# neel-dey/anatomix

Measured on AMD Instinct MI355X. Metric: 128^3 volumes/sec feature-extraction (6M UNet), higher is better.
Workload: dtype f16; 1 GPU; anatomix 6M UNet (ngf=16,num_downs=4) forward on sw_batch=4 windows of 1x128^3 (the predictor call of sliding_window_inference, BASELINE configs[1] / the metric); fp32 NCDHW in/out, 16-bit (f16) channels-last activations, fp32 accumulate; holds the 1e-3 tolerance against the fp32 reference in rel-L2 ONLY (max-norm 0.86e-3 .. 1.4e-3 by weight seed; the mode that holds both norms is value_strict); batch_per_gpu=4, window=128, parallelism=replicas x1 (no data-path collective)

## Files before the change

anatomix_amd/_lib.py:

```python
from __future__ import annotations

import ctypes as C
import os

_HERE = os.path.dirname(os.path.abspath(__file__))
LIB_PATH = os.environ.get("AMX_LIB_PATH") or os.path.join(_HERE, "csrc", "libanatomix_amd.so")

NORM = {"none": 0, "batch": 1, "instance": 2, "instance_affine": 3}
ACT = {"none": 0, "relu": 1, "lrelu": 2}
POOL = {"Max": 0, "Avg": 1}
INTERP = {"nearest": 0, "trilinear": 1}
WARP = {"bilinear": 0, "nearest": 1}
SEG_LABEL = {"float32": 0, "int64": 1, "uint8": 2}
SW_MAP = {"constant": 0, "gaussian": 1}
SW_OUT = {"features": 0, "logits": 1, "labels": 2}
PRECISION = {"f16": 0, "fp16": 0, "float16": 0, "bf16": 1, "bfloat16": 1, "f16x2": 2, "bf16x2": 3, "strict": 3, "fp32": 3,
             "f16x2mx": 4, "strict_mx": 4}


class UnetCfg(C.Structure):
    _fields_ = [
        ("input_nc", C.c_int32), ("output_nc", C.c_int32), ("num_downs", C.c_int32), ("ngf", C.c_int32),
        ("norm", C.c_int32), ("norm_eps", C.c_float), ("activation", C.c_int32), ("act_slope", C.c_float),
        ("final_act", C.c_int32), ("pooling", C.c_int32), ("interp", C.c_int32), ("doubleconv", C.c_int32),
# ... 62 lines not shown
    "amx_sliding_window_workspace_bytes": (C.c_size_t, [_P, _I, _I, _I, _I]),
    "amx_sliding_window": (_I, [_P, _P, _I, _I, _I, _I, _I, _I, C.c_double, _I, C.c_double, _I, _I, _P, _P, _I, _P, _P, _P, _P,
                                C.c_size_t, _P]),
    "amx_conv3d_packed_bytes": (C.c_size_t, [_I, _I]),
    "amx_conv3d_k3_reflect": (_I, [_P, _I, _P, _I, _P, _P, _P, _I, _I, _I, _I, _I, _I, C.c_float, _I, _P, _P, _P, _P]),
    "amx_conv3d_k3_reflect_probe": (_I, [_P, _I, _P, _I, _P, _P, _P, _I, _I, _I, _I, _I, _I, C.c_float, _I, _P, _P, _P, _P, _P, _P, _P, _P]),
    "amx_conv3d_dgrad_interior_supported": (_I, [_I, _I, _I, _I, _I, _I]),
    "amx_conv3d_dgrad_interior": (_I, [_P, _I, _P, _I, _I, _I, _I, _I, _I, _I, _I, _I, _P, _P, _P]),
    "amx_conv3d_dgrad_shell_scratch_bytes": (C.c_size_t, []),
    "amx_conv3d_dgrad_fold_shell": (_I, [_P, _I, _P, _I, _I, _P, _I, _I, _I, _I, _I, _I, _P, _P]),
    "amx_conv3d_pack_batch": (_I, [C.POINTER(PackReq), _I, _I, _P]),
    "amx_conv3d_scratch_bytes": (C.c_size_t, [_I, _I, _I, _I, _I, _I, _I, _I]),
    "amx_conv3d_k3_reflect_ws": (_I, [_P, _I, _P, _I, _P, _P, _P, _I, _I, _I, _I, _I, _I, C.c_float, _I, _P, _P, _P, _P, C.c_size_t, _P]),
    "amx_conv3d_upcat_merged_packed_bytes": (C.c_size_t, [_I, _I, _I]),
    "amx_conv3d_upcat_merged": (_I, [_P, _I, _P, _I, _P, _P, _P, _I, _I, _I, _I, _I, _I, C.c_float, _I, _P, _P, _P, _P]),
    "amx_conv3d_k3_reflect_ex": (_I, [_P, _I, _P, _I, _P, _I, _I, _I, _P, _P, _I, _I, _I, _I, _I, _I, C.c_float, _I, _P, _P, _P, _P]),
    "amx_pool2": (_I, [_P, _P, _I, _I, _I, _I, _I, _I, _I, _P]),
    "amx_instance_norm_scratch_bytes": (C.c_size_t, [_I, _I]),
    "amx_instance_norm": (_I, [_P, _P, _P, C.c_float, _I, C.c_longlong, _I, _I, C.c_float, _P, _I, _P]),
    "amx_upsample2_trilinear": (_I, [_P, _P, _I, _I, _I, _I, _I, _I, _P]),
    "amx_upsample2_trilinear_backward": (_I, [_P, _P, _I, _I, _I, _I, _I, _I, _P]),
    "amx_upcat_split_backward": (_I, [_P, _P, _P, _I, _I, _I, _I, _I, _I, _I, _I, _P]),
    "amx_upcat_split_backward_framed": (_I, [_P, _P, _P, _I, _I, _I, _I, _I, _I, _I, _I, _P]),
    "amx_export_ncdhw": (_I, [_P, _I, _I, _I, _I, _I, _P, _I, _P]),
    "amx_import_ncdhw": (_I, [_P, _P, _I, _I, _I, _I, _I, C.c_longlong, C.c_longlong, C.c_longlong, C.c_longlong, _I, _I, _P]),
    "amx_train_scratch_bytes": (C.c_size_t, [_I]),
    "amx_bn_train_forward": (_I, [_P, _P, _P, _P, C.c_float, _I, C.c_longlong, _I, _I, C.c_float, _P, _P, _P, _P, _P,
                                  C.c_float, _I, _P]),
    "amx_bn_act_backward": (_I, [_P, _P, _P, _P, _P, _P, _P, _P, _P, _I, _I, _I, _I, _I, _I, C.c_float, _P, _I, _P]),
    "amx_bn_act_backward_recompute": (_I, [_P, _P, _P, _P, _P, _P, _P, _P, _P, _I, _I, _I, _I, _I, _I, C.c_float, _P, _I, _P]),
# ... 183 lines not shown
```

anatomix_amd/csrc/amx_api.hip:

```cpp
#include <stdarg.h>
#include <stdio.h>
#include <string.h>

#include <string>
#include <vector>

#include "amx_gemm.h"
#include "amx_launch.h"

static thread_local std::string g_err;

int amx::fail(int code, const char* fmt, ...) {
  char buf[512];
  va_list ap;
  va_start(ap, fmt);
  vsnprintf(buf, sizeof buf, fmt, ap);
  va_end(ap);
  g_err = buf;
  return code;
}

using namespace amx;

extern "C" {
// ... 258 lines not shown
                       precision, d_wpk, d_out16, d_out32, stream);
}

int amx_conv3d_k3_reflect_ex(const void* d_x0, int c0, const void* d_x1, int c1, const float* d_weight, int weight_mode,
                             int cin_real, int cout_real, const float* d_scale, const float* d_shift, int cout, int n,
                             int d, int hh, int w, int act, float slope, int precision, void* d_wpk, void* d_out16,
                             float* d_out32, void* stream) {
  return conv3d_single(d_x0, c0, d_x1, c1, d_weight, weight_mode, cin_real, cout_real, d_scale, d_shift, cout, n, d, hh, w,
                       act, slope, precision, d_wpk, d_out16, d_out32, stream);
}

size_t amx_conv3d_upcat_merged_packed_bytes(int c0, int c1, int cout) {
  return 2 * (align_up((size_t)cout * c0 * 28 * 2, 256) + amx::conv_upmerge_packed_bytes(c1, cout, 0));
}

int amx_conv3d_upcat_merged(const void* d_x0, int c0, const void* d_x1, int c1, const float* d_weight, const float* d_scale,
                            const float* d_shift, int cout, int n, int d, int hh, int w, int act, float slope, int precision,
                            void* d_wpk, void* d_partial, void* d_out16, void* stream) {
  if (!d_x0 || !d_x1 || !d_weight || !d_wpk || !d_partial || !d_out16) return fail(AMX_ERR_INVALID, "null argument");
  if (precision < AMX_PREC_F16 || precision > AMX_PREC_BF16X2) return fail(AMX_ERR_INVALID, "unsupported precision %d", precision);
  const bool split = is_split(precision);
  if (c0 != cout || !amx::conv_upmerge_eligible(c0, c1, cout, d, hh, w, 1, split))
    return fail(AMX_ERR_INVALID, "merged concat conv needs c0 == cout >= 32 (16 in the strict precisions), c1 %% 32 == 0, w >= 16, even dims "
                "(c0=%d c1=%d cout=%d dims %d,%d,%d)", c0, c1, cout, d, hh, w);
  hipStream_t st = (hipStream_t)stream;
  const int q = amx::conv_pick_q(cout, w, precision);
  char* wmerge = (char*)d_wpk + align_up((size_t)cout * c0 * 28 * 2 * (split ? 2 : 1), 256);
  AMX_HIP(amx::launch_pack_weights(d_weight, d_scale, d_wpk, c0, c0, cout, q, precision, st, 0, 0, c0 + c1));
  AMX_HIP(amx::launch_pack_upmerge(d_weight, d_scale, wmerge, c0, c0 + c1, c1, cout, precision, st));
  amx::ConvParams p;
  memset(&p, 0, sizeof p);
  p.N = n; p.D = d; p.H = hh; p.W = w; p.Cout = cout;
  amx::set_src0(p, d_x0, c0, d, hh, w, precision);
  p.wpk = (const char*)d_wpk; p.act = AMX_ACT_NONE;
  amx::set_out(p, d_partial, cout, d, hh, w, precision);
  AMX_HIP(amx::launch_conv(p, precision, q, st));
  amx::UpmergeParams u;
  memset(&u, 0, sizeof u);
  amx::set_src(u, d_x1, c1, d / 2, hh / 2, w / 2, precision);
  u.N = n; u.LD = d / 2; u.LH = hh / 2; u.LW = w / 2; u.Cout = cout;
  u.wpk = wmerge; u.part = (const char*)d_partial; u.out = (char*)d_out16;
  u.bias = d_shift; u.act = act; u.slope = slope;
  AMX_HIP(amx::launch_conv_upmerge(u, precision, st));
  return AMX_OK;
}

int amx_pool2(const void* d_in, void* d_out, int n, int dout, int hout, int wout, int c, int avg, int precision,
              void* stream) {
  if (!d_in || !d_out || c % 8) return fail(AMX_ERR_INVALID, "bad argument");
  AMX_HIP(amx::launch_pool2(d_in, d_out, n, dout, hout, wout, c, avg, precision, (hipStream_t)stream));
  return AMX_OK;
}

size_t amx_train_scratch_bytes(int c) { return amx::train_scratch_bytes(c); }

int amx_bn_train_forward(const void* d_x, void* d_y, const float* d_gamma, const float* d_beta, float eps, int n,
                         long long voxels, int c, int act, float slope, void* d_scratch, float* d_save_mean,
                         float* d_save_rstd, float* d_running_mean, float* d_running_var, float momentum, int precision,
                         void* stream) {
// ... 600 lines not shown
```

anatomix_amd/csrc/amx_common.h:

```cpp
#pragma once
#include <hip/hip_runtime.h>
#include <stdint.h>
#include <stdlib.h>

namespace amx {

typedef _Float16 f16;
typedef __bf16 bf16;
typedef __attribute__((ext_vector_type(8))) _Float16 f16x8;
typedef __attribute__((ext_vector_type(8))) __bf16 bf16x8;
typedef __attribute__((ext_vector_type(4))) float f32x4;

constexpr int kSteps = 14;

__host__ __device__ constexpr int tapA_index(int s) {
  return s < 9 ? s * 3 : (s < 12 ? (s - 9) * 9 + 2 : (s == 12 ? 8 : 26));
}
__host__ __device__ constexpr int tapB_index(int s) {
  return s < 9 ? s * 3 + 1 : (s < 12 ? (s - 9) * 9 + 5 : (s == 12 ? 17 : -1));
}

enum Act { ACT_NONE = 0, ACT_RELU = 1, ACT_LRELU = 2 };

struct DeviceOnce {
// ... 64 lines not shown
}

struct UpmergeParams {
  const char* src;
  long long sn, sz, sy, sx;
  int C1;
  int N, LD, LH, LW, Cout;
  const char* wpk;
  const char* part;
  char* out;
  const float* bias;
  int act;
  float slope;
  int nbz, nby, nbx;
  int* oflow;
  int dbg;
  int cs, ocs;
};

constexpr int MLP_MAXB = 8;

struct WgradParams {
  const char* dy;
  long long yn, yz, yy, yx;
  const char* src0;
  long long s0n, s0z, s0y, s0x;
  const char* src1;
  long long s1n, s1z, s1y, s1x;
  int C0, C1, up_shift;
  int N, D, H, W, Cout;
  float* partial;
// ... 9 lines not shown
```

anatomix_amd/csrc/amx_conv3d_upmerge.hip:

```cpp
#include <stdlib.h>

#include "amx_device.h"
#include "amx_launch.h"

namespace amx {


template <int Q, int TZ, int TY, int NBUF, int KS, bool SPLIT = false, int LXT = 16>
struct UpmCfg {
  static_assert(LXT == 16 || LXT == 8, "a tile is 16 cells of one low-res row, or 8 cells of two rows (rows shorter than 16)");
  static constexpr int RPT = 16 / LXT;
  static constexpr int BY = TY * RPT;
  static constexpr int NP = SPLIT ? 2 : 1;
  static_assert(!SPLIT || KS == 1, "strict precision: 32-channel stages");
  static constexpr int T = TZ * TY;
  static constexpr int HZ = TZ + 2, HY = BY + 2, HX = LXT + 2, HV = HZ * HY * HX;
  static constexpr int PL = ((HV * 16 + 255) / 256) * 256;
  static constexpr int BUF = 4 * KS * NP * PL;
  static constexpr int NJ = (HV + 63) / 64;
  static constexpr int NDMA = 4 * KS * NP * NJ;
  static constexpr int PER_WAVE = (NDMA + 7) / 8;
  static constexpr int LDS_BYTES = NBUF * BUF;
  static_assert(LDS_BYTES <= 160 * 1024, "ring must fit the LDS");
};

template <typename T_, int Q, int TZ, int TY, int NBUF, int KS, bool SPLIT, int LXT>
__global__ __launch_bounds__(512) void conv3d_upmerge_kernel(const UpmergeParams p) {
  typedef UpmCfg<Q, TZ, TY, NBUF, KS, SPLIT, LXT> C;
  constexpr int RPT = C::RPT, BY = C::BY;
  constexpr int NP = C::NP;
  typedef typename Ops<T_>::vec8 vec8;
  constexpr int HY = C::HY, HX = C::HX, PL = C::PL, NT = C::T;
  extern __shared__ __attribute__((aligned(16))) char smem[];

  const int tid = threadIdx.x, lane = tid & 63;
  const int wave = __builtin_amdgcn_readfirstlane(tid >> 6);
  const int li = lane & 15, g = lane >> 4;
  const int lix = li & (LXT - 1), liy = LXT == 8 ? li >> 3 : 0;
  const int pz = wave >> 2, py = (wave >> 1) & 1, px = wave & 1;

  const int nbricks = p.nbz * p.nby * p.nbx * p.N;
  const int ncg = p.Cout / (16 * Q);
  const int items = nbricks * ncg;
  const int G = gridDim.x;
  int jw = blockIdx.x;
  if ((G & 7) == 0) jw = (jw & 7) * (G >> 3) + (jw >> 3);
  const int it0 = (int)((long long)items * jw / G), it1 = (int)((long long)items * (jw + 1) / G);
  const int nstage = p.C1 / (32 * KS);
  const int T_total = (it1 - it0) * nstage;
  if (T_total <= 0) return;

  struct Item { int bx, by, bz, n, cg; };
  auto decode = [&](int it) {
    Item r;
    r.cg = it / nbricks;
    int b = it - r.cg * nbricks;
    r.bx = b % p.nbx; b /= p.nbx;
    r.by = b % p.nby; b /= p.nby;
    r.bz = b % p.nbz;
    r.n = b / p.nbz;
    return r;
  };

  int dma_item = -1;
  int off[C::PER_WAVE];
  auto issue = [&](int it, int stage, int bsel) {
    const Item I = decode(it);
    if (it != dma_item) {
      dma_item = it;
#pragma unroll
      for (int m = 0; m < C::PER_WAVE; ++m) {
        const int id = wave + 8 * m;
        const int j = id % C::NJ;
        const int hv = j * 64 + lane;
        const int hz = hv / (HY * HX), rem = hv - hz * (HY * HX), hy = rem / HX, hx = rem - hy * HX;
        int gz = I.bz * TZ - 1 + hz, gy = I.by * BY - 1 + hy, gx = I.bx * LXT - 1 + hx;
        gz = gz < 0 ? 0 : (gz >= p.LD ? p.LD - 1 : gz);
        gy = gy < 0 ? 0 : (gy >= p.LH ? p.LH - 1 : gy);
        gx = gx < 0 ? 0 : (gx >= p.LW ? p.LW - 1 : gx);
        off[m] = hv < C::HV ? gz * (int)p.sz + gy * (int)p.sy + gx * (int)p.sx : -1;
      }
    }
    const char* base = p.src + (long long)I.n * p.sn;
    const int cs = p.cs ? p.cs : 32;
    char* buf = smem + bsel * C::BUF;
#pragma unroll
    for (int m = 0; m < C::PER_WAVE; ++m) {
      const int id = wave + 8 * m;
      if (id < C::NDMA) {
        const int plane = id / C::NJ, j = id - plane * C::NJ;
        const int cbyte = stage * (64 * KS) + (SPLIT && plane >= 4 ? p.C1 * 2 + (plane - 4) * 16 : plane * 16);
        if (off[m] >= 0)
          dma16_asm(base + off[m] + (long long)(cbyte >> 5) * cs + (cbyte & 31),
                    (unsigned)__builtin_amdgcn_readfirstlane((int)lds_addr(buf + plane * PL + j * 1024)));
      }
    }
  };

  auto wptr = [&](int it, int stage) -> const char* {
    const int cg = it / nbricks;
    return p.wpk + ((((long long)cg * nstage * KS + stage * KS) * 8 + wave) * 8 * NP * Q) * 1024 + lane * 16;
  };
  auto woff = [](const int e2) { return ((e2 >> 3) * 64 + (e2 & 7)) * NP * Q * 1024; };
  constexpr int NTAP = 8 * KS;
  constexpr int WIN = 4;
  vec8 wq[WIN][NP][Q];
  const int lbase = g * PL + ((pz * HY + py + liy) * HX + px + lix) * 16;

  f32x4 acc[NT][Q];
  int nx_it = it0, nx_stage = 0;
  auto step_next = [&]() {
    if (++nx_stage == nstage) { nx_stage = 0; ++nx_it; }
  };
  issue(nx_it, nx_stage, 0);
  step_next();
  if (NBUF > 2 && T_total > 1) { issue(nx_it, nx_stage, 1); step_next(); }
  {
    const char* w0 = wptr(it0, 0);
#pragma unroll
    for (int e = 0; e < WIN; ++e)
#pragma unroll
      for (int h = 0; h < NP; ++h)
#pragma unroll
        for (int q = 0; q < Q; ++q) wq[e][h][q] = *(const vec8*)(w0 + woff(e) + (h * Q + q) * 1024);
  }

  int cu_it = it0, cu_stage = 0;
  bool bad = false;
  unsigned pend[NT][2 * Q * NP];
  int pend_it = -1;
  unsigned padd[NT][2 * Q * NP];
  auto load_part = [&](const int it) {
    const Item I = decode(it);
    const int lx = I.bx * LXT + lix;
    const int ocs = p.ocs ? p.ocs : 32, cb2 = (I.cg * 16 * Q + g * 4 * Q) * 2;
    const long long sy = (long long)p.Cout * 2 * NP * (2 * p.LW), sz = sy * (2 * p.LH), sx = ocs == 32 ? (long long)p.Cout * 2 * NP : 32;
    const char* pb = p.part + (long long)I.n * sz * (2 * p.LD) + pz * sz + py * sy + (2 * lx + px) * sx + (long long)(cb2 >> 5) * ocs + (cb2 & 31);
#pragma unroll
    for (int i = 0; i < NT; ++i) {
      const int lz = I.bz * TZ + i / TY, ly = I.by * BY + (i % TY) * RPT + liy;
      const bool in = (lz < p.LD) & (ly < p.LH) & (lx < p.LW);
#pragma unroll
      for (int hl = 0; hl < NP; ++hl) {
        const char* src = pb + 2 * lz * sz + 2 * ly * sy + hl * p.Cout * 2;
        unsigned* dst = &padd[i][hl * 2 * Q];
        if (Q == 1) {
          const uint2 v = in ? *(const uint2*)src : make_uint2(0u, 0u);
          dst[0] = v.x; dst[1] = v.y;
        } else {
#pragma unroll
          for (int h = 0; h < Q / 2; ++h) {
            const uint4 v = in ? *(const uint4*)(src + h * 16) : make_uint4(0u, 0u, 0u, 0u);
            dst[4 * h] = v.x; dst[4 * h + 1] = v.y; dst[4 * h + 2] = v.z; dst[4 * h + 3] = v.w;
          }
        }
      }
    }
  };
  auto flush = [&]() {
    const Item I = decode(pend_it);
    pend_it = -1;
    const int lx = I.bx * LXT + lix;
    const int ocs = p.ocs ? p.ocs : 32, cb2 = (I.cg * 16 * Q + g * 4 * Q) * 2;
    const long long sy = (long long)p.Cout * 2 * NP * (2 * p.LW), sz = sy * (2 * p.LH), sx = ocs == 32 ? (long long)p.Cout * 2 * NP : 32;
    char* pb = p.out + (long long)I.n * sz * (2 * p.LD) + pz * sz + py * sy + (2 * lx + px) * sx + (long long)(cb2 >> 5) * ocs + (cb2 & 31);
#pragma unroll
    for (int i = 0; i < NT; ++i) {
      const int lz = I.bz * TZ + i / TY, ly = I.by * BY + (i % TY) * RPT + liy;
      if (lz >= p.LD || ly >= p.LH || lx >= p.LW) continue;
#pragma unroll
      for (int hl = 0; hl < NP; ++hl) {
        char* dst = pb + 2 * lz * sz + 2 * ly * sy + hl * p.Cout * 2;
        const unsigned* v = &pend[i][hl * 2 * Q];
        if (Q == 1) *(uint2*)dst = make_uint2(v[0], v[1]);
        else {
#pragma unroll
          for (int h = 0; h < Q / 2; ++h) *(uint4*)(dst + h * 16) = make_uint4(v[4 * h], v[4 * h + 1], v[4 * h + 2], v[4 * h + 3]);
        }
      }
    }
  };
  for (int t = 0; t < T_total; ++t) {
    if (t == 0) asm volatile("s_waitcnt vmcnt(0)" ::: "memory");
    else asm volatile("" ::"v"(wq[0][0][0]) : "memory");
    __syncthreads();
    if (t + NBUF - 1 < T_total && !(p.dbg & 1)) {
      issue(nx_it, nx_stage, (t + NBUF - 1) % NBUF);
      step_next();
    }
    if (pend_it >= 0 && !(p.dbg & 4)) flush();
    if (cu_stage == nstage - 1 && !(p.dbg & 16)) load_part(cu_it);
    const char* buf = smem + (t % NBUF) * C::BUF + lbase;
    if (cu_stage == 0) {
#pragma unroll
      for (int i = 0; i < NT; ++i)
#pragma unroll
        for (int q = 0; q < Q; ++q) acc[i][q] = f32x4{0.f, 0.f, 0.f, 0.f};
    }
    const bool more = t + 1 < T_total;
    const int w_it = cu_stage + 1 < nstage ? cu_it : cu_it + 1, w_stage = cu_stage + 1 < nstage ? cu_stage + 1 : 0;
    const char* wn = more ? wptr(w_it, w_stage) : p.wpk;
    const char* wc = wptr(cu_it, cu_stage);
    if (!(p.dbg & 2)) {
      constexpr int GT = SPLIT ? 2 : (NT < 4 ? NT : 4), NGT = NT / GT, NG = NTAP * NGT;
      vec8 fb[2][GT][NP];
      auto load_group = [&](const int gi, const int set) {
        const int e2 = gi / NGT, i0 = (gi % NGT) * GT;
        const int ks = e2 >> 3, ez = (e2 >> 2) & 1, ey = (e2 >> 1) & 1, ex = e2 & 1;
#pragma unroll
        for (int k = 0; k < GT; ++k) {
          const int lz = (i0 + k) / TY, ly = (i0 + k) % TY;
#pragma unroll
          for (int h = 0; h < NP; ++h)
            fb[set][k][h] = *(const vec8*)(buf + (ks + h) * 4 * PL + (((lz + ez) * HY + ly * RPT + ey) * HX + ex) * 16);
        }
      };
      load_group(0, 0);
#pragma unroll
// ... 12 lines not shown
            }
          }
        __builtin_amdgcn_sched_barrier(0);
        if ((gi % NGT) == NGT - 1 && (e + WIN < NTAP || more)) {
          const char* src = e + WIN < NTAP ? wc + woff(e + WIN) : wn + woff(e + WIN - NTAP);
#pragma unroll
          for (int h = 0; h < NP; ++h)
#pragma unroll
            for (int q = 0; q < Q; ++q) wq[e % WIN][h][q] = *(const vec8*)(src + (h * Q + q) * 1024);
        }
      }
    }
    if (++cu_stage < nstage) continue;
    cu_stage = 0;

    {
      const int cgb = (cu_it / nbricks) * 16 * Q + g * 4 * Q;
      auto cvt = [](const unsigned w, const int half) { return (float)__builtin_bit_cast(T_, (unsigned short)(half ? w >> 16 : w & 0xffffu)); };
#pragma unroll
      for (int q = 0; q < Q; ++q) {
        const f32x4 bv = p.bias ? *(const f32x4*)(p.bias + cgb + q * 4) : f32x4{0.f, 0.f, 0.f, 0.f};
#pragma unroll
        for (int i = 0; i < NT; ++i)
#pragma unroll
          for (int j = 0; j < 4; ++j) {
            float a = cvt(padd[i][2 * q + (j >> 1)], j & 1);
            if (SPLIT) a += cvt(padd[i][2 * Q + 2 * q + (j >> 1)], j & 1);
            acc[i][q][j] += bv[j] + a;
          }
      }
      act_inplace<NT * Q>(&acc[0][0], p.act, p.slope);
    }
#pragma unroll
    for (int i = 0; i < NT; ++i)
#pragma unroll
      for (int q = 0; q < Q; ++q) {
#pragma unroll
        for (int j = 0; j < 4; ++j)
          if (RangeCheck<T_>::on) bad |= RangeCheck<T_>::bad(acc[i][q][j]);
        pend[i][2 * q] = (unsigned)to_bits<T_>(acc[i][q][0]) | ((unsigned)to_bits<T_>(acc[i][q][1]) << 16);
        pend[i][2 * q + 1] = (unsigned)to_bits<T_>(acc[i][q][2]) | ((unsigned)to_bits<T_>(acc[i][q][3]) << 16);
        if (SPLIT) {
          float r[4];
#pragma unroll
          for (int j = 0; j < 4; ++j) r[j] = acc[i][q][j] - (float)(T_)acc[i][q][j];
          pend[i][2 * Q + 2 * q] = (unsigned)to_bits<T_>(r[0]) | ((unsigned)to_bits<T_>(r[1]) << 16);
          pend[i][2 * Q + 2 * q + 1] = (unsigned)to_bits<T_>(r[2]) | ((unsigned)to_bits<T_>(r[3]) << 16);
        }
      }
    pend_it = cu_it;
    ++cu_it;
  }
  if (pend_it >= 0 && !(p.dbg & 4)) flush();
  if (RangeCheck<T_>::on) raise_flag(p.oflow, bad);
}

template <typename T>
__global__ void pack_upmerge_kernel(const float* __restrict__ w, const float* __restrict__ scale, T* __restrict__ wpk, int c_off,
                                    int CinTotal, int C1, int Cout, int Q, int split) {
  const int nstage = C1 / 32, NP = split ? 2 : 1;
  const long long total = (long long)(Cout / (16 * Q)) * nstage * 64 * NP * Q * 512;
  for (long long idx = blockIdx.x * (long long)blockDim.x + threadIdx.x; idx < total; idx += (long long)gridDim.x * blockDim.x) {
    const int j = idx & 7, lane = (idx >> 3) & 63;
    long long r = idx >> 9;
    const int q = r % Q; r /= Q;
    const int part = r % NP; r /= NP;
    const int e = r % 8; r /= 8;
    const int cls = r % 8; r /= 8;
// ... 16 lines not shown
    const float v = sum * (scale ? scale[cout] : 1.f);
    const T vh = (T)v;
    wpk[idx] = part ? (T)(v - (float)vh) : vh;
  }
}

size_t conv_upmerge_packed_bytes(int C1, int Cout, int split) { return (size_t)Cout * C1 * 64 * 2 * (split ? 2 : 1); }
size_t conv_upmerge_partial_bytes(int N, int D, int H, int W, int Cout) { return (size_t)N * D * H * W * Cout * 2; }
int conv_upmerge_q(int Cout, int split) { return (!split && Cout % 32 == 0) ? 2 : 1; }

bool conv_upmerge_eligible(int C0, int C1, int Cout, int D, int H, int W, int up_shift, int split) {
  return up_shift == 1 && C0 >= 16 && C1 >= 32 && C1 % 32 == 0 && Cout >= (split ? 16 : 32) && Cout % 16 == 0 && W >= 16 && !(D & 1) && !(H & 1) &&
         !(W & 1) && D >= 4 && H >= 4;
}

template <typename T, int Q, int TZ, int TY, int NBUF, int KS, bool SPLIT = false, int LXT = 16>
static hipError_t launch_upm(UpmergeParams p, hipStream_t st, ConvLaunchInfo* info) {
  typedef UpmCfg<Q, TZ, TY, NBUF, KS, SPLIT, LXT> C;
  if (info)
    info->report(0, "conv3d_upmerge<%s,q%d,%dx%dx%d,b%d,k%d>", __is_same(T, f16) ? (SPLIT ? "f16x2" : "f16") : (SPLIT ? "bf16x2" : "bf16"), Q,
                 TZ, C::BY, LXT, NBUF, 32 * KS);
  auto kern = conv3d_upmerge_kernel<T, Q, TZ, TY, NBUF, KS, SPLIT, LXT>;
  static amx::DeviceOnce attr_once;
  if (!attr_once.done()) {
    hipError_t e = hipFuncSetAttribute((const void*)kern, hipFuncAttributeMaxDynamicSharedMemorySize, C::LDS_BYTES);
    if (e != hipSuccess) return e;
    attr_once.set();
  }
  const int cus = device_cus(attr_once.dev);
  if (cus == 0) return hipErrorUnknown;
  p.nbz = (p.LD + TZ - 1) / TZ;
  p.nby = (p.LH + C::BY - 1) / C::BY;
  p.nbx = (p.LW + LXT - 1) / LXT;
  const long long items = (long long)p.nbz * p.nby * p.nbx * p.N * (p.Cout / (16 * Q));
  const long long grid = items < cus ? items : cus;
  hipLaunchKernelGGL(kern, dim3((unsigned)grid), dim3(512), C::LDS_BYTES, st, p);
  return hipGetLastError();
}

template <typename T>
static hipError_t launch_upm_split(const UpmergeParams& p, hipStream_t st, ConvLaunchInfo* info) {
  if (p.LW < 16) return launch_upm<T, 1, 2, 2, 3, 1, true, 8>(p, st, info);
  const long long cells = (long long)p.N * p.LD * p.LH * ((p.LW + 15) / 16);
  if (cells / 8 * (p.Cout / 16) >= 256) return launch_upm<T, 1, 2, 4, 2, 1, true>(p, st, info);
  return launch_upm<T, 1, 2, 2, 3, 1, true>(p, st, info);
}

template <typename T>
static hipError_t launch_upm_t(const UpmergeParams& p, hipStream_t st, ConvLaunchInfo* info) {
  const int Q = conv_upmerge_q(p.Cout, 0);
  if (p.LW < 16) {
    if (Q == 2) return p.C1 % 64 == 0 ? launch_upm<T, 2, 2, 2, 2, 2, false, 8>(p, st, info) : launch_upm<T, 2, 2, 2, 3, 1, false, 8>(p, st, info);
// ... 36 lines not shown
```

include/anatomix_amd.h:

```cpp
#ifndef ANATOMIX_AMD_H
#define ANATOMIX_AMD_H

#include <stddef.h>
#include <stdint.h>

#ifdef __cplusplus
extern "C" {
#endif

#define AMX_VERSION 100

typedef enum amx_status {
  AMX_OK = 0,
  AMX_ERR_INVALID = -1,
  AMX_ERR_SHAPE = -2,
  AMX_ERR_NOT_LOADED = -3,
  AMX_ERR_WORKSPACE = -4,
  AMX_ERR_HIP = -5,
  AMX_ERR_OVERFLOW = -6
} amx_status;

enum { AMX_NORM_NONE = 0, AMX_NORM_BATCH_EVAL = 1, AMX_NORM_INSTANCE = 2, AMX_NORM_INSTANCE_AFFINE = 3 };
enum { AMX_ACT_NONE = 0, AMX_ACT_RELU = 1, AMX_ACT_LRELU = 2 };
enum { AMX_POOL_MAX = 0, AMX_POOL_AVG = 1 };
// ... 155 lines not shown
int amx_upcat_split_backward_framed(const void* d_g_framed, void* d_dskip, void* d_dlow, int n, int dlow, int hlow, int wlow, int c0,
                                    int c1, int accumulate_skip, int precision, void* stream);

int amx_import_input(const float* d_src, void* d_dst, int n, int cin, int d, int hh, int w, int precision, void* stream);
int amx_export_ncdhw(const void* d_src, int c, int n, int d, int hh, int w, float* d_out, int precision, void* stream);
int amx_import_ncdhw(const float* d_src, void* d_dst, int n, int c, int d, int hh, int w, long long dst_sn, long long dst_sz,
                     long long dst_sy, long long dst_sx, int accumulate, int precision, void* stream);

int amx_upsample2_trilinear_backward(const void* d_gout, void* d_gin, int n, int din, int hin, int win, int c, int precision,
                                     void* stream);

size_t amx_conv3d_upcat_merged_packed_bytes(int c0, int c1, int cout);
int amx_conv3d_upcat_merged(const void* d_x0, int c0, const void* d_x1, int c1, const float* d_weight, const float* d_scale,
                            const float* d_shift, int cout, int n, int d, int hh, int w, int act, float slope, int precision,
                            void* d_wpk, void* d_partial, void* d_out16, void* stream);

size_t amx_train_scratch_bytes(int c);

int amx_bn_train_forward(const void* d_x, void* d_y, const float* d_gamma, const float* d_beta, float eps, int n,
                         long long voxels, int c, int act, float slope, void* d_scratch, float* d_save_mean,
                         float* d_save_rstd, float* d_running_mean, float* d_running_var, float momentum, int precision,
                         void* stream);

int amx_bn_act_backward(const void* d_dy, const void* d_y, const void* d_x, const float* d_mean, const float* d_rstd,
                        const float* d_gamma, float* d_dgamma, float* d_dbeta, void* d_dx_framed, int n, int d, int hh, int w,
                        int c, int act, float slope, void* d_scratch, int precision, void* stream);
int amx_bn_act_backward_recompute(const void* d_dy, const void* d_x, const float* d_mean, const float* d_rstd, const float* d_gamma,
                                  const float* d_beta, float* d_dgamma, float* d_dbeta, void* d_dx_framed, int n, int d, int hh, int w,
                                  int c, int act, float slope, void* d_scratch, int precision, void* stream);

// ... 410 lines not shown
```

Before: 3049 volumes/s.

## Stage upmerge partial/output through an LDS tile with async DMA for non-split f16

For the non-split Q=2 upmerge conv, the partial-sum input is loaded into an LDS item tile with async DMA, the epilogue is applied in place, and the tile is written out coalesced in the next step. This replaces per-thread strided register loads and stores of the partial and output. The change also specializes the activation at compile time, precomputes halo coordinates, and advances items incrementally instead of decoding them with divisions. It uses more LDS and adds extra barriers, and it also adds a probe entry point and drops the debug flags.

After: 3043 volumes/s. About the same (-0.2%).

```diff
diff --git a/anatomix_amd/_lib.py b/anatomix_amd/_lib.py
--- a/anatomix_amd/_lib.py
+++ b/anatomix_amd/_lib.py
@@ -100,6 +100,7 @@
     "amx_conv3d_k3_reflect_ws": (_I, [_P, _I, _P, _I, _P, _P, _P, _I, _I, _I, _I, _I, _I, C.c_float, _I, _P, _P, _P, _P, C.c_size_t, _P]),
     "amx_conv3d_upcat_merged_packed_bytes": (C.c_size_t, [_I, _I, _I]),
     "amx_conv3d_upcat_merged": (_I, [_P, _I, _P, _I, _P, _P, _P, _I, _I, _I, _I, _I, _I, C.c_float, _I, _P, _P, _P, _P]),
+    "amx_conv3d_upcat_merged_probe": (_I, [_P, _I, _P, _I, _P, _P, _P, _I, _I, _I, _I, _I, _I, C.c_float, _I, _P, _P, _P, _P, _P, _P]),
     "amx_conv3d_k3_reflect_ex": (_I, [_P, _I, _P, _I, _P, _I, _I, _I, _P, _P, _I, _I, _I, _I, _I, _I, C.c_float, _I, _P, _P, _P, _P]),
     "amx_pool2": (_I, [_P, _P, _I, _I, _I, _I, _I, _I, _I, _P]),
     "amx_instance_norm_scratch_bytes": (C.c_size_t, [_I, _I]),
diff --git a/anatomix_amd/csrc/amx_api.hip b/anatomix_amd/csrc/amx_api.hip
--- a/anatomix_amd/csrc/amx_api.hip
+++ b/anatomix_amd/csrc/amx_api.hip
@@ -296,9 +296,14 @@
   return 2 * (align_up((size_t)cout * c0 * 28 * 2, 256) + amx::conv_upmerge_packed_bytes(c1, cout, 0));
 }
 
-int amx_conv3d_upcat_merged(const void* d_x0, int c0, const void* d_x1, int c1, const float* d_weight, const float* d_scale,
-                            const float* d_shift, int cout, int n, int d, int hh, int w, int act, float slope, int precision,
-                            void* d_wpk, void* d_partial, void* d_out16, void* stream) {
+struct MergedProbe {
+  int* oflow;
+  char* kernel;
+};
+
+static int conv3d_upcat_merged(const void* d_x0, int c0, const void* d_x1, int c1, const float* d_weight, const float* d_scale,
+                               const float* d_shift, int cout, int n, int d, int hh, int w, int act, float slope, int precision,
+                               void* d_wpk, void* d_partial, void* d_out16, void* stream, const MergedProbe* probe = nullptr) {
   if (!d_x0 || !d_x1 || !d_weight || !d_wpk || !d_partial || !d_out16) return fail(AMX_ERR_INVALID, "null argument");
   if (precision < AMX_PREC_F16 || precision > AMX_PREC_BF16X2) return fail(AMX_ERR_INVALID, "unsupported precision %d", precision);
   const bool split = is_split(precision);
@@ -323,8 +328,26 @@
   u.N = n; u.LD = d / 2; u.LH = hh / 2; u.LW = w / 2; u.Cout = cout;
   u.wpk = wmerge; u.part = (const char*)d_partial; u.out = (char*)d_out16;
   u.bias = d_shift; u.act = act; u.slope = slope;
-  AMX_HIP(amx::launch_conv_upmerge(u, precision, st));
-  return AMX_OK;
+  amx::ConvLaunchInfo info{};
+  if (probe) u.oflow = probe->oflow;
+  AMX_HIP(amx::launch_conv_upmerge(u, precision, st, probe ? &info : nullptr));
+  if (probe && probe->kernel) memcpy(probe->kernel, info.name, sizeof info.name);
+  return AMX_OK;
+}
+
+int amx_conv3d_upcat_merged(const void* d_x0, int c0, const void* d_x1, int c1, const float* d_weight, const float* d_scale,
+                            const float* d_shift, int cout, int n, int d, int hh, int w, int act, float slope, int precision,
+                            void* d_wpk, void* d_partial, void* d_out16, void* stream) {
+  return conv3d_upcat_merged(d_x0, c0, d_x1, c1, d_weight, d_scale, d_shift, cout, n, d, hh, w, act, slope, precision, d_wpk, d_partial,
+                             d_out16, stream);
+}
+
+int amx_conv3d_upcat_merged_probe(const void* d_x0, int c0, const void* d_x1, int c1, const float* d_weight, const float* d_scale,
+                                  const float* d_shift, int cout, int n, int d, int hh, int w, int act, float slope, int precision,
+                                  void* d_wpk, void* d_partial, void* d_out16, int* d_oflow, char* kernel_name, void* stream) {
+  const MergedProbe probe{d_oflow, kernel_name};
+  return conv3d_upcat_merged(d_x0, c0, d_x1, c1, d_weight, d_scale, d_shift, cout, n, d, hh, w, act, slope, precision, d_wpk, d_partial,
+                             d_out16, stream, &probe);
 }
 
 int amx_pool2(const void* d_in, void* d_out, int n, int dout, int hout, int wout, int c, int avg, int precision,
diff --git a/anatomix_amd/csrc/amx_common.h b/anatomix_amd/csrc/amx_common.h
--- a/anatomix_amd/csrc/amx_common.h
+++ b/anatomix_amd/csrc/amx_common.h
@@ -102,7 +102,6 @@
   float slope;
   int nbz, nby, nbx;
   int* oflow;
-  int dbg;
   int cs, ocs;
 };
 
diff --git a/anatomix_amd/csrc/amx_conv3d_upmerge.hip b/anatomix_amd/csrc/amx_conv3d_upmerge.hip
--- a/anatomix_amd/csrc/amx_conv3d_upmerge.hip
+++ b/anatomix_amd/csrc/amx_conv3d_upmerge.hip
@@ -20,15 +20,25 @@
   static constexpr int NJ = (HV + 63) / 64;
   static constexpr int NDMA = 4 * KS * NP * NJ;
   static constexpr int PER_WAVE = (NDMA + 7) / 8;
-  static constexpr int LDS_BYTES = NBUF * BUF;
-  static_assert(LDS_BYTES <= 160 * 1024, "ring must fit the LDS");
+  static constexpr int RING_BYTES = NBUF * BUF;
+  static constexpr bool STAGED = !SPLIT && Q == 2;
+  static constexpr int ZB = 2 * TZ, YB = 2 * BY, XV = 2 * LXT;
+  static constexpr int TILE_BYTES = STAGED ? ZB * YB * XV * 64 : 0;
+  static constexpr int TPW = TILE_BYTES / (512 * 16);
+  static_assert(!STAGED || (TILE_BYTES % (512 * 16) == 0 && XV >= 16), "a DMA instruction covers 16 voxels of one row");
+  static constexpr int LDS_BYTES = RING_BYTES + TILE_BYTES;
+  static_assert(LDS_BYTES <= 160 * 1024, "ring and item tile must fit the LDS");
 };
-
-template <typename T_, int Q, int TZ, int TY, int NBUF, int KS, bool SPLIT, int LXT>
+static_assert(UpmCfg<2, 2, 4, 3, 1>::TILE_BYTES == 64 * 1024 && UpmCfg<2, 2, 4, 3, 1>::RING_BYTES <= 83 * 1024, "96 -> 32: 64 KiB beside 83 KiB");
+static_assert(UpmCfg<2, 2, 2, 2, 2, false, 8>::TILE_BYTES == 32 * 1024 && UpmCfg<2, 2, 2, 2, 2, false, 8>::RING_BYTES <= 61 * 1024,
+              "384 -> 128 @16: 32 KiB beside 61 KiB");
+
+template <typename T_, int Q, int TZ, int TY, int NBUF, int KS, bool SPLIT, int LXT, int ACT>
 __global__ __launch_bounds__(512) void conv3d_upmerge_kernel(const UpmergeParams p) {
   typedef UpmCfg<Q, TZ, TY, NBUF, KS, SPLIT, LXT> C;
   constexpr int RPT = C::RPT, BY = C::BY;
   constexpr int NP = C::NP;
+  constexpr bool STAGED = C::STAGED;
   typedef typename Ops<T_>::vec8 vec8;
   constexpr int HY = C::HY, HX = C::HX, PL = C::PL, NT = C::T;
   extern __shared__ __attribute__((aligned(16))) char smem[];
@@ -50,38 +60,54 @@
   const int T_total = (it1 - it0) * nstage;
   if (T_total <= 0) return;
 
-  struct Item { int bx, by, bz, n, cg; };
+  struct Item { int bx, by, bz, n, cg, b; };
   auto decode = [&](int it) {
     Item r;
     r.cg = it / nbricks;
-    int b = it - r.cg * nbricks;
+    int b = r.b = it - r.cg * nbricks;
     r.bx = b % p.nbx; b /= p.nbx;
     r.by = b % p.nby; b /= p.nby;
     r.bz = b % p.nbz;
     r.n = b / p.nbz;
     return r;
   };
-
-  int dma_item = -1;
+  auto advance = [&](Item& r) {
+    if (++r.b == nbricks) { r.b = r.bx = r.by = r.bz = r.n = 0; ++r.cg; return; }
+    if (++r.bx < p.nbx) return;
+    r.bx = 0;
+    if (++r.by < p.nby) return;
+    r.by = 0;
+    if (++r.bz < p.nbz) return;
+    r.bz = 0;
+    ++r.n;
+  };
+
+  int hpk[C::PER_WAVE];
+#pragma unroll
+  for (int m = 0; m < C::PER_WAVE; ++m) {
+    const int id = wave + 8 * m;
+    const int j = id % C::NJ;
+    const int hv = j * 64 + lane;
+    const int hz = hv / (HY * HX), rem = hv - hz * (HY * HX), hy = rem / HX, hx = rem - hy * HX;
+    hpk[m] = hv < C::HV ? (hz << 16) | (hy << 8) | hx : -1;
+  }
   int off[C::PER_WAVE];
-  auto issue = [&](int it, int stage, int bsel) {
-    const Item I = decode(it);
-    if (it != dma_item) {
-      dma_item = it;
+  Item nx = decode(it0);
+  int nx_stage = 0;
+  bool nx_fresh = true;
+  auto issue = [&](int bsel) {
+    if (nx_fresh) {
+      nx_fresh = false;
 #pragma unroll
       for (int m = 0; m < C::PER_WAVE; ++m) {
-        const int id = wave + 8 * m;
-        const int j = id % C::NJ;
-        const int hv = j * 64 + lane;
-        const int hz = hv / (HY * HX), rem = hv - hz * (HY * HX), hy = rem / HX, hx = rem - hy * HX;
-        int gz = I.bz * TZ - 1 + hz, gy = I.by * BY - 1 + hy, gx = I.bx * LXT - 1 + hx;
+        int gz = nx.bz * TZ - 1 + (hpk[m] >> 16), gy = nx.by * BY - 1 + ((hpk[m] >> 8) & 255), gx = nx.bx * LXT - 1 + (hpk[m] & 255);
         gz = gz < 0 ? 0 : (gz >= p.LD ? p.LD - 1 : gz);
         gy = gy < 0 ? 0 : (gy >= p.LH ? p.LH - 1 : gy);
         gx = gx < 0 ? 0 : (gx >= p.LW ? p.LW - 1 : gx);
-        off[m] = hv < C::HV ? gz * (int)p.sz + gy * (int)p.sy + gx * (int)p.sx : -1;
-      }
-    }
-    const char* base = p.src + (long long)I.n * p.sn;
+        off[m] = hpk[m] >= 0 ? gz * (int)p.sz + gy * (int)p.sy + gx * (int)p.sx : -1;
+      }
+    }
+    const char* base = p.src + (long long)nx.n * p.sn;
     const int cs = p.cs ? p.cs : 32;
     char* buf = smem + bsel * C::BUF;
 #pragma unroll
@@ -89,16 +115,16 @@
       const int id = wave + 8 * m;
       if (id < C::NDMA) {
         const int plane = id / C::NJ, j = id - plane * C::NJ;
-        const int cbyte = stage * (64 * KS) + (SPLIT && plane >= 4 ? p.C1 * 2 + (plane - 4) * 16 : plane * 16);
+        const int cbyte = nx_stage * (64 * KS) + (SPLIT && plane >= 4 ? p.C1 * 2 + (plane - 4) * 16 : plane * 16);
         if (off[m] >= 0)
           dma16_asm(base + off[m] + (long long)(cbyte >> 5) * cs + (cbyte & 31),
                     (unsigned)__builtin_amdgcn_readfirstlane((int)lds_addr(buf + plane * PL + j * 1024)));
       }
     }
-  };
-
-  auto wptr = [&](int it, int stage) -> const char* {
-    const int cg = it / nbricks;
+    if (++nx_stage == nstage) { nx_stage = 0; advance(nx); nx_fresh = true; }
+  };
+
+  auto wptr = [&](int cg, int stage) -> const char* {
     return p.wpk + ((((long long)cg * nstage * KS + stage * KS) * 8 + wave) * 8 * NP * Q) * 1024 + lane * 16;
   };
   auto woff = [](const int e2) { return ((e2 >> 3) * 64 + (e2 & 7)) * NP * Q * 1024; };
@@ -108,15 +134,12 @@
   const int lbase = g * PL + ((pz * HY + py + liy) * HX + px + lix) * 16;
 
   f32x4 acc[NT][Q];
-  int nx_it = it0, nx_stage = 0;
-  auto step_next = [&]() {
-    if (++nx_stage == nstage) { nx_stage = 0; ++nx_it; }
-  };
-  issue(nx_it, nx_stage, 0);
-  step_next();
-  if (NBUF > 2 && T_total > 1) { issue(nx_it, nx_stage, 1); step_next(); }
+  issue(0);
+  if (NBUF > 2 && T_total > 1) issue(1);
+  Item cu = decode(it0);
+  int cu_stage = 0;
   {
-    const char* w0 = wptr(it0, 0);
+    const char* w0 = wptr(cu.cg, 0);
 #pragma unroll
     for (int e = 0; e < WIN; ++e)
 #pragma unroll
@@ -125,24 +148,75 @@
         for (int q = 0; q < Q; ++q) wq[e][h][q] = *(const vec8*)(w0 + woff(e) + (h * Q + q) * 1024);
   }
 
-  int cu_it = it0, cu_stage = 0;
   bool bad = false;
-  unsigned pend[NT][2 * Q * NP];
-  int pend_it = -1;
-  unsigned padd[NT][2 * Q * NP];
-  auto load_part = [&](const int it) {
-    const Item I = decode(it);
+  const int ocs = p.ocs ? p.ocs : 32;
+  const long long osy = (long long)p.Cout * 2 * NP * (2 * p.LW), osz = osy * (2 * p.LH), osx = ocs == 32 ? (long long)p.Cout * 2 * NP : 32;
+
+  char* const tile = smem + C::RING_BYTES;
+  struct Io { long long base; int zl, yl, xl; };
+  auto io_of = [&](const Item& I) {
+    Io r;
+    const int z0 = I.bz * C::ZB, y0 = I.by * C::YB, x0 = I.bx * C::XV;
+    r.base = (long long)I.n * osz * (2 * p.LD) + z0 * osz + y0 * osy + x0 * osx + I.cg * 64;
+    r.zl = 2 * p.LD - z0; r.yl = 2 * p.LH - y0; r.xl = 2 * p.LW - x0;
+    return r;
+  };
+  const int lpo_c = (lane >> 2) * (int)osx + (lane & 3) * 16;
+  auto piece = [&](const int m, int& tz, int& ty, int& tx) {
+    const int v = (wave + 8 * m) * 16;
+    tx = v & (C::XV - 1); ty = (v / C::XV) & (C::YB - 1); tz = v / (C::XV * C::YB);
+  };
+  auto part_in = [&](const Io& io) {
+    int lpo = lpo_c;
+    asm volatile("" : "+v"(lpo));
+#pragma unroll
+    for (int m = 0; m < C::TPW; ++m) {
+      int tz, ty, tx;
+      piece(m, tz, ty, tx);
+      if (tz < io.zl && ty < io.yl && tx + (lane >> 2) < io.xl)
+        dma16_asm(p.part + (io.base + tz * osz + ty * osy + tx * osx) + lpo,
+                  (unsigned)__builtin_amdgcn_readfirstlane((int)lds_addr(tile + (wave + 8 * m) * 1024)));
+    }
+  };
+  auto tile_out = [&](const Io& io) {
+    int lpo = lpo_c;
+    asm volatile("" : "+v"(lpo));
+    uint4 v[C::TPW > 0 ? C::TPW : 1];
+#pragma unroll
+    for (int m = 0; m < C::TPW; ++m) v[m] = *(const uint4*)(tile + (wave + 8 * m) * 1024 + lane * 16);
+#pragma unroll
+    for (int m = 0; m < C::TPW; ++m) {
+      int tz, ty, tx;
+      piece(m, tz, ty, tx);
+      if (tz < io.zl && ty < io.yl && tx + (lane >> 2) < io.xl) *(uint4*)(p.out + (io.base + tz * osz + ty * osy + tx * osx) + lpo) = v[m];
+    }
+  };
+  const int tslot = ((pz * C::YB + 2 * liy + py) * C::XV + 2 * lix + px) * 64 + g * 16;
+  Io cu_io = io_of(cu), out_io = cu_io;
+  bool out_pend = false;
+  const int part_stage = nstage > 1 ? 1 : 0;
+  if constexpr (STAGED) part_in(cu_io);
+
+  constexpr int NREG = STAGED ? 1 : NT;
+  unsigned pend[NREG][2 * Q * NP];
+  unsigned padd[NREG][2 * Q * NP];
+  Item pend_I = cu;
+  bool pend_on = false;
+  auto row_ptr = [&](const char* t, const Item& I) {
     const int lx = I.bx * LXT + lix;
-    const int ocs = p.ocs ? p.ocs : 32, cb2 = (I.cg * 16 * Q + g * 4 * Q) * 2;
-    const long long sy = (long long)p.Cout * 2 * NP * (2 * p.LW), sz = sy * (2 * p.LH), sx = ocs == 32 ? (long long)p.Cout * 2 * NP : 32;
-    const char* pb = p.part + (long long)I.n * sz * (2 * p.LD) + pz * sz + py * sy + (2 * lx + px) * sx + (long long)(cb2 >> 5) * ocs + (cb2 & 31);
-#pragma unroll
-    for (int i = 0; i < NT; ++i) {
+    const int cb2 = (I.cg * 16 * Q + g * 4 * Q) * 2;
+    return t + (long long)I.n * osz * (2 * p.LD) + pz * osz + py * osy + (2 * lx + px) * osx + (long long)(cb2 >> 5) * ocs + (cb2 & 31);
+  };
+  auto load_part = [&](const Item& I) {
+    const int lx = I.bx * LXT + lix;
+    const char* pb = row_ptr(p.part, I);
+#pragma unroll
+    for (int i = 0; i < NREG; ++i) {
       const int lz = I.bz * TZ + i / TY, ly = I.by * BY + (i % TY) * RPT + liy;
       const bool in = (lz < p.LD) & (ly < p.LH) & (lx < p.LW);
 #pragma unroll
       for (int hl = 0; hl < NP; ++hl) {
-        const char* src = pb + 2 * lz * sz + 2 * ly * sy + hl * p.Cout * 2;
+        const char* src = pb + 2 * lz * osz + 2 * ly * osy + hl * p.Cout * 2;
         unsigned* dst = &padd[i][hl * 2 * Q];
         if (Q == 1) {
           const uint2 v = in ? *(const uint2*)src : make_uint2(0u, 0u);
@@ -158,19 +232,17 @@
     }
   };
   auto flush = [&]() {
-    const Item I = decode(pend_it);
-    pend_it = -1;
+    const Item& I = pend_I;
+    pend_on = false;
     const int lx = I.bx * LXT + lix;
-    const int ocs = p.ocs ? p.ocs : 32, cb2 = (I.cg * 16 * Q + g * 4 * Q) * 2;
-    const long long sy = (long long)p.Cout * 2 * NP * (2 * p.LW), sz = sy * (2 * p.LH), sx = ocs == 32 ? (long long)p.Cout * 2 * NP : 32;
-    char* pb = p.out + (long long)I.n * sz * (2 * p.LD) + pz * sz + py * sy + (2 * lx + px) * sx + (long long)(cb2 >> 5) * ocs + (cb2 & 31);
-#pragma unroll
-    for (int i = 0; i < NT; ++i) {
+    char* pb = const_cast<char*>(row_ptr(p.out, I));
+#pragma unroll
+    for (int i = 0; i < NREG; ++i) {
       const int lz = I.bz * TZ + i / TY, ly = I.by * BY + (i % TY) * RPT + liy;
       if (lz >= p.LD || ly >= p.LH || lx >= p.LW) continue;
 #pragma unroll
       for (int hl = 0; hl < NP; ++hl) {
-        char* dst = pb + 2 * lz * sz + 2 * ly * sy + hl * p.Cout * 2;
+        char* dst = pb + 2 * lz * osz + 2 * ly * osy + hl * p.Cout * 2;
         const unsigned* v = &pend[i][hl * 2 * Q];
         if (Q == 1) *(uint2*)dst = make_uint2(v[0], v[1]);
         else {
@@ -180,16 +252,23 @@
       }
     }
   };
+  auto cvt = [](const unsigned w, const int half) { return (float)__builtin_bit_cast(T_, (unsigned short)(half ? w >> 16 : w & 0xffffu)); };
   for (int t = 0; t < T_total; ++t) {
     if (t == 0) asm volatile("s_waitcnt vmcnt(0)" ::: "memory");
     else asm volatile("" ::"v"(wq[0][0][0]) : "memory");
     __syncthreads();
-    if (t + NBUF - 1 < T_total && !(p.dbg & 1)) {
-      issue(nx_it, nx_stage, (t + NBUF - 1) % NBUF);
-      step_next();
-    }
-    if (pend_it >= 0 && !(p.dbg & 4)) flush();
-    if (cu_stage == nstage - 1 && !(p.dbg & 16)) load_part(cu_it);
+    if (t + NBUF - 1 < T_total) issue((t + NBUF - 1) % NBUF);
+    if constexpr (STAGED) {
+      if (out_pend) {
+        out_pend = false;
+        tile_out(out_io);
+        if (nstage == 1) __syncthreads();
+      }
+      if (t >= nstage && cu_stage == part_stage) part_in(cu_io);
+    } else {
+      if (pend_on) flush();
+      if (cu_stage == nstage - 1) load_part(cu);
+    }
     const char* buf = smem + (t % NBUF) * C::BUF + lbase;
     if (cu_stage == 0) {
 #pragma unroll
@@ -198,10 +277,10 @@
         for (int q = 0; q < Q; ++q) acc[i][q] = f32x4{0.f, 0.f, 0.f, 0.f};
     }
     const bool more = t + 1 < T_total;
-    const int w_it = cu_stage + 1 < nstage ? cu_it : cu_it + 1, w_stage = cu_stage + 1 < nstage ? cu_stage + 1 : 0;
-    const char* wn = more ? wptr(w_it, w_stage) : p.wpk;
-    const char* wc = wptr(cu_it, cu_stage);
-    if (!(p.dbg & 2)) {
+    const int w_cg = cu_stage + 1 < nstage ? cu.cg : cu.cg + (cu.b + 1 == nbricks), w_stage = cu_stage + 1 < nstage ? cu_stage + 1 : 0;
+    const char* wn = more ? wptr(w_cg, w_stage) : p.wpk;
+    const char* wc = wptr(cu.cg, cu_stage);
+    {
       constexpr int GT = SPLIT ? 2 : (NT < 4 ? NT : 4), NGT = NT / GT, NG = NTAP * NGT;
       vec8 fb[2][GT][NP];
       auto load_group = [&](const int gi, const int set) {
@@ -244,9 +323,44 @@
     if (++cu_stage < nstage) continue;
     cu_stage = 0;
 
-    {
-      const int cgb = (cu_it / nbricks) * 16 * Q + g * 4 * Q;
-      auto cvt = [](const unsigned w, const int half) { return (float)__builtin_bit_cast(T_, (unsigned short)(half ? w >> 16 : w & 0xffffu)); };
+    const int cgb = cu.cg * 16 * Q + g * 4 * Q;
+    if constexpr (STAGED) {
+      if (more) asm volatile("" ::"v"(wq[0][0][0]) : "memory");
+      else asm volatile("s_waitcnt vmcnt(0)" ::: "memory");
+      __syncthreads();
+      const int lx = cu.bx * LXT + lix;
+      f32x4 bv[Q];
+#pragma unroll
+      for (int q = 0; q < Q; ++q) bv[q] = p.bias ? *(const f32x4*)(p.bias + cgb + q * 4) : f32x4{0.f, 0.f, 0.f, 0.f};
+#pragma unroll
+      for (int i = 0; i < NT; ++i) {
+        uint4* slot = (uint4*)(tile + tslot + ((2 * (i / TY) * C::YB + 2 * (i % TY) * RPT) * C::XV) * 64);
+        const int lz = cu.bz * TZ + i / TY, ly = cu.by * BY + (i % TY) * RPT + liy;
+        const bool in = (lz < p.LD) & (ly < p.LH) & (lx < p.LW);
+        const uint4 r = *slot;
+        const unsigned w[4] = {in ? r.x : 0u, in ? r.y : 0u, in ? r.z : 0u, in ? r.w : 0u};
+#pragma unroll
+        for (int q = 0; q < Q; ++q)
+#pragma unroll
+          for (int j = 0; j < 4; ++j) acc[i][q][j] += bv[q][j] + cvt(w[2 * q + (j >> 1)], j & 1);
+        act_values<ACT, Q>(&acc[i][0], p.slope);
+        unsigned o[4];
+#pragma unroll
+        for (int q = 0; q < Q; ++q) {
+#pragma unroll
+          for (int j = 0; j < 4; ++j)
+            if (RangeCheck<T_>::on) bad |= RangeCheck<T_>::bad(acc[i][q][j]);
+          o[2 * q] = (unsigned)to_bits<T_>(acc[i][q][0]) | ((unsigned)to_bits<T_>(acc[i][q][1]) << 16);
+          o[2 * q + 1] = (unsigned)to_bits<T_>(acc[i][q][2]) | ((unsigned)to_bits<T_>(acc[i][q][3]) << 16);
+        }
+        *slot = make_uint4(o[0], o[1], o[2], o[3]);
+        if (i & 1) __builtin_amdgcn_sched_barrier(0);
+      }
+      out_io = cu_io;
+      out_pend = true;
+      advance(cu);
+      cu_io = io_of(cu);
+    } else {
 #pragma unroll
       for (int q = 0; q < Q; ++q) {
         const f32x4 bv = p.bias ? *(const f32x4*)(p.bias + cgb + q * 4) : f32x4{0.f, 0.f, 0.f, 0.f};
@@ -259,29 +373,37 @@
             acc[i][q][j] += bv[j] + a;
           }
       }
-      act_inplace<NT * Q>(&acc[0][0], p.act, p.slope);
-    }
-#pragma unroll
-    for (int i = 0; i < NT; ++i)
-#pragma unroll
-      for (int q = 0; q < Q; ++q) {
-#pragma unroll
-        for (int j = 0; j < 4; ++j)
-          if (RangeCheck<T_>::on) bad |= RangeCheck<T_>::bad(acc[i][q][j]);
-        pend[i][2 * q] = (unsigned)to_bits<T_>(acc[i][q][0]) | ((unsigned)to_bits<T_>(acc[i][q][1]) << 16);
-        pend[i][2 * q + 1] = (unsigned)to_bits<T_>(acc[i][q][2]) | ((unsigned)to_bits<T_>(acc[i][q][3]) << 16);
-        if (SPLIT) {
-          float r[4];
-#pragma unroll
-          for (int j = 0; j < 4; ++j) r[j] = acc[i][q][j] - (float)(T_)acc[i][q][j];
-          pend[i][2 * Q + 2 * q] = (unsigned)to_bits<T_>(r[0]) | ((unsigned)to_bits<T_>(r[1]) << 16);
-          pend[i][2 * Q + 2 * q + 1] = (unsigned)to_bits<T_>(r[2]) | ((unsigned)to_bits<T_>(r[3]) << 16);
+      act_values<ACT, NT * Q>(&acc[0][0], p.slope);
+#pragma unroll
+      for (int i = 0; i < NT; ++i)
+#pragma unroll
+        for (int q = 0; q < Q; ++q) {
+#pragma unroll
+          for (int j = 0; j < 4; ++j)
+            if (RangeCheck<T_>::on) bad |= RangeCheck<T_>::bad(acc[i][q][j]);
+          pend[i][2 * q] = (unsigned)to_bits<T_>(acc[i][q][0]) | ((unsigned)to_bits<T_>(acc[i][q][1]) << 16);
+          pend[i][2 * q + 1] = (unsigned)to_bits<T_>(acc[i][q][2]) | ((unsigned)to_bits<T_>(acc[i][q][3]) << 16);
+          if (SPLIT) {
+            float r[4];
+#pragma unroll
+            for (int j = 0; j < 4; ++j) r[j] = acc[i][q][j] - (float)(T_)acc[i][q][j];
+            pend[i][2 * Q + 2 * q] = (unsigned)to_bits<T_>(r[0]) | ((unsigned)to_bits<T_>(r[1]) << 16);
+            pend[i][2 * Q + 2 * q + 1] = (unsigned)to_bits<T_>(r[2]) | ((unsigned)to_bits<T_>(r[3]) << 16);
+          }
         }
-      }
-    pend_it = cu_it;
-    ++cu_it;
-  }
-  if (pend_it >= 0 && !(p.dbg & 4)) flush();
+      pend_I = cu;
+      pend_on = true;
+      advance(cu);
+    }
+  }
+  if constexpr (STAGED) {
+    if (out_pend) {
+      __syncthreads();
+      tile_out(out_io);
+    }
+  } else {
+    if (pend_on) flush();
+  }
   if (RangeCheck<T_>::on) raise_flag(p.oflow, bad);
 }
 
@@ -328,13 +450,10 @@
          !(W & 1) && D >= 4 && H >= 4;
 }
 
-template <typename T, int Q, int TZ, int TY, int NBUF, int KS, bool SPLIT = false, int LXT = 16>
-static hipError_t launch_upm(UpmergeParams p, hipStream_t st, ConvLaunchInfo* info) {
+template <typename T, int Q, int TZ, int TY, int NBUF, int KS, bool SPLIT, int LXT, int ACT>
+static hipError_t launch_upm_act(UpmergeParams p, hipStream_t st) {
   typedef UpmCfg<Q, TZ, TY, NBUF, KS, SPLIT, LXT> C;
-  if (info)
-    info->report(0, "conv3d_upmerge<%s,q%d,%dx%dx%d,b%d,k%d>", __is_same(T, f16) ? (SPLIT ? "f16x2" : "f16") : (SPLIT ? "bf16x2" : "bf16"), Q,
-                 TZ, C::BY, LXT, NBUF, 32 * KS);
-  auto kern = conv3d_upmerge_kernel<T, Q, TZ, TY, NBUF, KS, SPLIT, LXT>;
+  auto kern = conv3d_upmerge_kernel<T, Q, TZ, TY, NBUF, KS, SPLIT, LXT, ACT>;
   static amx::DeviceOnce attr_once;
   if (!attr_once.done()) {
     hipError_t e = hipFuncSetAttribute((const void*)kern, hipFuncAttributeMaxDynamicSharedMemorySize, C::LDS_BYTES);
@@ -343,6 +462,7 @@
   }
   const int cus = device_cus(attr_once.dev);
   if (cus == 0) return hipErrorUnknown;
+  if (C::STAGED && ((p.ocs != 0 && p.ocs != 32) || (long long)p.Cout * 2 * (2 * p.LW) * (2 * p.LH) * (2 * TZ) >= (1ll << 31))) return hipErrorInvalidValue;
   p.nbz = (p.LD + TZ - 1) / TZ;
   p.nby = (p.LH + C::BY - 1) / C::BY;
   p.nbx = (p.LW + LXT - 1) / LXT;
@@ -350,6 +470,17 @@
   const long long grid = items < cus ? items : cus;
   hipLaunchKernelGGL(kern, dim3((unsigned)grid), dim3(512), C::LDS_BYTES, st, p);
   return hipGetLastError();
+}
+
+template <typename T, int Q, int TZ, int TY, int NBUF, int KS, bool SPLIT = false, int LXT = 16>
+static hipError_t launch_upm(const UpmergeParams& p, hipStream_t st, ConvLaunchInfo* info) {
+  typedef UpmCfg<Q, TZ, TY, NBUF, KS, SPLIT, LXT> C;
+  if (info)
+    info->report(0, "conv3d_upmerge<%s,q%d,%dx%dx%d,b%d,k%d>", __is_same(T, f16) ? (SPLIT ? "f16x2" : "f16") : (SPLIT ? "bf16x2" : "bf16"), Q,
+                 TZ, C::BY, LXT, NBUF, 32 * KS);
+  if (p.act == ACT_RELU) return launch_upm_act<T, Q, TZ, TY, NBUF, KS, SPLIT, LXT, ACT_RELU>(p, st);
+  if (p.act == ACT_LRELU) return launch_upm_act<T, Q, TZ, TY, NBUF, KS, SPLIT, LXT, ACT_LRELU>(p, st);
+  return launch_upm_act<T, Q, TZ, TY, NBUF, KS, SPLIT, LXT, ACT_NONE>(p, st);
 }
 
 template <typename T>
diff --git a/include/anatomix_amd.h b/include/anatomix_amd.h
--- a/include/anatomix_amd.h
+++ b/include/anatomix_amd.h
@@ -193,6 +193,9 @@
 int amx_conv3d_upcat_merged(const void* d_x0, int c0, const void* d_x1, int c1, const float* d_weight, const float* d_scale,
                             const float* d_shift, int cout, int n, int d, int hh, int w, int act, float slope, int precision,
                             void* d_wpk, void* d_partial, void* d_out16, void* stream);
+int amx_conv3d_upcat_merged_probe(const void* d_x0, int c0, const void* d_x1, int c1, const float* d_weight, const float* d_scale,
+                                  const float* d_shift, int cout, int n, int d, int hh, int w, int act, float slope, int precision,
+                                  void* d_wpk, void* d_partial, void* d_out16, int* d_oflow, char* kernel_name, void* stream);
 
 size_t amx_train_scratch_bytes(int c);
 
```
